# Samaretas/global-motion-estimation

Measured on AMD Instinct MI355X. Metric: frame-pairs/s + achieved HBM GB/s, 720x480 bs=16 sw=16 exhaustive, higher is better.
Workload: dtype u8; 1 GPU; 720x480 synthetic luma, bs=16 sw=16 exhaustive MAE (BASELINE configs[1]); frame_distance=1, streams_per_gpu=1, collective=none, exchange=none in this run, multi_gpu_measured_by_builder=False

## Files before the change

global-motion-estimation_amd/csrc/bbme_sea.hip:

```cpp
#include "bbme_sea_common.h"

namespace {

using namespace sea;

constexpr int GUARD_NONE = 0, GUARD_ROWS = 1, GUARD_ALL = 2;
constexpr uint32_t PENALTY = 1u << 17;
constexpr uint32_t FIRST_INVALID_KEY = 65536u << 13;
constexpr uint32_t FIRST_INVALID_BOUND = FIRST_INVALID_KEY >> 13;
__device__ __forceinline__ uint32_t pair_u16(uint32_t t, uint32_t b, bool odd)
{
    return __builtin_amdgcn_perm(b, t, odd ? 0x07060302u : 0x05040100u);
}
template <bool VERT>
__device__ __forceinline__ void candidate_pairs(uint32_t tl, uint32_t tr, uint32_t bl, uint32_t br, bool odd, uint32_t* first, uint32_t* second)
{
    *first = VERT ? pair_u16(tl, bl, odd) : pair_u16(tl, tr, odd);
    *second = VERT ? pair_u16(tr, br, odd) : pair_u16(bl, br, odd);
}
template <int R, int GUARD, bool VERT>
__device__ __forceinline__ void lower_bounds(const uint64_t* sp0, int XQ, int prow, int q, uint32_t pa, uint32_t pb,
                                             int lo_r, int hi_r, int lo_c, int hi_c, uint32_t (&pmin)[R])
{
    constexpr bool SKIP = GUARD == GUARD_ALL && R >= 4;
#pragma unroll
    for (int k = 0; k < R; ++k) pmin[k] = 0xFFFFFFFFu;
    constexpr uint32_t penalty = PENALTY;
    uint32_t seed[R];
#pragma unroll
    for (int i = 0; i < R; ++i) {
        const int ri = prow * R + i;
        seed[i] = (GUARD == GUARD_NONE || SKIP || (ri >= lo_r && ri <= hi_r)) ? 0u : penalty;
    }
    const int nlo = lo_c - q * 4 * R, nhi = hi_c - q * 4 * R;
    const uint64_t* top = sp0;
    const uint64_t* bot = sp0 + 8 * XQ;
#pragma unroll
    for (int i = 0; i < R; ++i) {
        const int ri = prow * R + i;
        if (!SKIP || (ri >= lo_r && ri <= hi_r)) {
            uint64_t t[R + 2], b[R + 2];
#pragma unroll
            for (int k = 0; k < R + 2; ++k) { t[k] = top[k]; b[k] = bot[k]; }
            if constexpr (SKIP || !VERT) {
#pragma unroll
                for (int k = 0; k < R; ++k) {
                    if (SKIP && (4 * k > nhi || 4 * k + 3 < nlo)) continue;
#pragma unroll
                    for (int e = 0; e < 4; ++e) {
                        if (SKIP && (4 * k + e < nlo || 4 * k + e > nhi)) continue;
                        const int sh = 32 * (e >> 1);
                        uint32_t first, second;
                        candidate_pairs<VERT>((uint32_t)(t[k] >> sh), (uint32_t)(t[k + 2] >> sh), (uint32_t)(b[k] >> sh), (uint32_t)(b[k + 2] >> sh), e & 1, &first, &second);
                        const uint32_t start = (GUARD != GUARD_ALL || SKIP || 4 * k + e <= nhi) ? seed[i] : penalty;
                        pmin[k] = min(pmin[k], __builtin_amdgcn_sad_u16(first, pa, __builtin_amdgcn_sad_u16(second, pb, start)));
                    }
                }
            } else {
                uint32_t vp[R + 2][4];
#pragma unroll
                for (int k = 0; k < R; ++k) {
#pragma unroll
                    for (int m = (k < 2 ? k : k + 2); m <= k + 2; m += 2)
#pragma unroll
                        for (int e = 0; e < 4; ++e)
                            vp[m][e] = pair_u16((uint32_t)(t[m] >> (32 * (e >> 1))), (uint32_t)(b[m] >> (32 * (e >> 1))), e & 1);
                    uint32_t lb[4];
#pragma unroll
                    for (int e = 0; e < 4; ++e) {
                        const uint32_t start = (GUARD != GUARD_ALL || 4 * k + e <= nhi) ? seed[i] : penalty;
                        lb[e] = __builtin_amdgcn_sad_u16(vp[k][e], pa, __builtin_amdgcn_sad_u16(vp[k + 2][e], pb, start));
                    }
                    pmin[k] = min(min(pmin[k], lb[0]), lb[1]);
                    pmin[k] = min(min(pmin[k], lb[2]), lb[3]);
                }
            }
        }
        top += XQ;
        bot += XQ;
    }
    if constexpr (GUARD != GUARD_NONE && !SKIP) {
#pragma unroll
        for (int k = 0; k < R; ++k)
            if (pmin[k] >= FIRST_INVALID_BOUND || (GUARD == GUARD_ALL && 4 * k < nlo)) pmin[k] = 0xFFFFFFFFu;
    }
}

template <int R, bool VERT>
__device__ __forceinline__ int min_bound_candidate(const uint64_t* s8blk, int XQ, int NC, int bl, uint32_t mb, uint32_t pa, uint32_t pb,
                                                   int lo_r, int hi_r, int lo_c, int hi_c, int lane)
{
    const int col0 = (bl & 3) * 4 * R, row0 = (bl >> 2) * R;
    const uint16_t* tab = (const uint16_t*)(s8blk + row0 * XQ + (bl & 3) * R);
    int loc = 0;
    bool found = false;
#pragma unroll
    for (int base = 0; base < 4 * R * R; base += 64) {
        const int l = base + lane;
        const int ce = l / R, li = l - ce * R;
        bool hit = false;
        if (4 * R * R - base >= 64 || l < 4 * R * R) {
            const uint16_t* p = tab + li * 4 * XQ + ce;
            uint32_t first, second;
            candidate_pairs<VERT>(p[0], p[8], p[32 * XQ], p[32 * XQ + 8], false, &first, &second);
            const uint32_t lb = __builtin_amdgcn_sad_u16(first, pa, __builtin_amdgcn_sad_u16(second, pb, 0u));
            const int ci = col0 + ce, ri = row0 + li;
            hit = lb == mb && ci >= lo_c && ci <= hi_c && ri >= lo_r && ri <= hi_r;
        }
        const unsigned long long m = __ballot(hit);
        if (!found && m) {
            loc = base + __builtin_ctzll(m);
            found = true;
        }
    }
    const int ce = loc / R, li = loc - ce * R;
    return (col0 + ce) * NC + row0 + li;
}

template <int R>
__device__ __forceinline__ uint32_t eval_patch_quad(const SeaGeo& d, int H, int W, const uint32_t* win, const uint32_t* anchor, uint32_t ent,
                                                    bool active, int sub, int trow, int bcol0, int NC)
{
    const int w2 = ent >> 25, l2 = (ent >> 19) & 63, k2 = (ent >> 16) & 7;
    const int wr2 = div_small(w2, d.magic_tc), wc2 = w2 - wr2 * d.tc;
    const int prow2 = l2 >> 2, q2 = l2 & 3;
    uint64_t acc[R];
#pragma unroll
    for (int i = 0; i < R; ++i) acc[i] = 0;
    if (active) {
        const uint32_t* lrow = win + (16 * wr2 + prow2 * R + 4 * sub) * d.pitch_dw + wc2 * 4 + q2 * R + k2;
        const uint32_t* an = anchor + w2 * ANCHOR_STRIDE + 16 * sub;
#pragma unroll
        for (int t = 0; t < R + 3; ++t) {
            uint64_t w[4];
#pragma unroll
            for (int s = 0; s < 4; ++s) w[s] = *(const u64_a4*)(lrow + t * d.pitch_dw + s);
#pragma unroll
            for (int i = 0; i < R; ++i) {
                const int a = t - i;
                if (a < 0 || a > 3) continue;
                const u32x4 ar = *(const u32x4*)(an + a * 4);
#pragma unroll
                for (int j = 0; j < 4; ++j)
                    acc[i] = __builtin_amdgcn_qsad_pk_u16_u8(w[j], ar[j], acc[i]);
            }
        }
    }
#pragma unroll
    for (int i = 0; i < R; ++i) {
        uint32_t lo = (uint32_t)acc[i], hi = (uint32_t)(acc[i] >> 32);
        lo += (uint32_t)__builtin_amdgcn_update_dpp(0, (int)lo, 0xB1, 0xF, 0xF, false);
        hi += (uint32_t)__builtin_amdgcn_update_dpp(0, (int)hi, 0xB1, 0xF, 0xF, false);
        lo += (uint32_t)__builtin_amdgcn_update_dpp(0, (int)lo, 0x4E, 0xF, 0xF, false);
        hi += (uint32_t)__builtin_amdgcn_update_dpp(0, (int)hi, 0x4E, 0xF, 0xF, false);
        asm volatile("" : "+v"(lo), "+v"(hi));
        acc[i] = ((uint64_t)hi << 32) | lo;
    }
    uint32_t key = 0xFFFFFFFFu;
    if (active) {
        const int c02 = (bcol0 + wc2) * 16, r02 = (trow * d.tr + wr2) * 16;
        const int lo_c = max(0, d.sw - c02), hi_c = min(NC - 1, W - 16 - c02 + d.sw);
        const int lo_r2 = max(0, d.sw - r02), hi_r2 = min(NC - 1, H - 16 - r02 + d.sw);
        const bool rows_inside2 = NC == 16 * R && lo_r2 == 0 && hi_r2 == NC - 1;
        const int ci = q2 * 4 * R + 4 * k2 + sub, ri0 = prow2 * R;
        const uint32_t shift = (uint32_t)(sub & 1) * 16u;
        if (rows_inside2 && lo_c == 0 && hi_c == NC - 1) {
#pragma unroll
            for (int i = 0; i < R; ++i) {
                const uint32_t word = (sub & 2) ? (uint32_t)(acc[i] >> 32) : (uint32_t)acc[i];
                const uint32_t sad = __builtin_amdgcn_ubfe(word, shift, 16u);
                key = min(key, (sad << 13) + (uint32_t)i);
            }
            key += (uint32_t)(ci * NC + ri0);
        } else if (ci >= lo_c && ci <= hi_c) {
#pragma unroll
            for (int i = 0; i < R; ++i) {
                const int ri = ri0 + i;
                if (ri < lo_r2 || ri > hi_r2) continue;
                const uint32_t word = (sub & 2) ? (uint32_t)(acc[i] >> 32) : (uint32_t)acc[i];
                const uint32_t sad = __builtin_amdgcn_ubfe(word, shift, 16u);
                key = min(key, (sad << 13) | (uint32_t)(ci * NC + ri));
            }
        }
        key = min(key, (uint32_t)__builtin_amdgcn_update_dpp(-1, (int)key, 0xB1, 0xF, 0xF, false));
        key = min(key, (uint32_t)__builtin_amdgcn_update_dpp(-1, (int)key, 0x4E, 0xF, 0xF, false));
    }
    return key;
}

template <int R, bool FIXED, bool VERT>
__device__ __forceinline__ bool tile_phases(const SeaGeo& d, uint32_t* lds, const Layout& L, int pair, int trow, int bcol0,
                                            uint32_t mine, uint32_t pa, uint32_t pb, int tid, int tile_id)
{
    constexpr bool E4 = R >= 3;
    const int T = blockDim.x;
    const int NC = 2 * d.sw + 16, XQ = d.xq;
    uint32_t* win = lds + L.win;
    uint32_t* anchor = lds + L.anchor;
    uint32_t* best = lds + L.best;
    uint32_t* count = lds + L.count;
    uint64_t* s8 = (uint64_t*)(lds + L.s8);
    uint32_t* work = lds + L.work;
    const int wave = __builtin_amdgcn_readfirstlane(tid >> 6);
    const int lane = tid & 63;
    const SeaArgs c = launch_args();
    const WaveBlock wb = wave_block(d, c, trow, bcol0, wave);
    const int brow = wb.brow, bcol = wb.bcol;
    const bool wave_ok = wb.ok;
    const int r0 = brow * 16, c0 = bcol * 16;
    const int prow = lane >> 2, q = lane & 3;

    box_sums8<R, FIXED>(d, win, s8, tid);
    __syncthreads();

    const int lo_r = max(0, d.sw - r0), hi_r = min(NC - 1, c->H - 16 - r0 + d.sw);
    const bool rows_inside = NC == 16 * R && lo_r == 0 && hi_r == NC - 1;
    uint32_t ub_key = 0xFFFFFFFFu;
    if (wave_ok) {
        const int lo_c = max(0, d.sw - c0), hi_c = min(NC - 1, c->W - 16 - c0 + d.sw);
        uint32_t pmin[R];
        const uint64_t* s8blk = s8 + 16 * wb.wr * XQ + wb.wc * 4;
        const uint64_t* sp0 = s8blk + prow * R * XQ + q * R;
        const bool cols_inside = NC == 16 * R && lo_c == 0 && hi_c == NC - 1;
        if (rows_inside && cols_inside)
            lower_bounds<R, GUARD_NONE, VERT>(sp0, XQ, prow, q, pa, pb, lo_r, hi_r, lo_c, hi_c, pmin);
        else if (R <= 3 && cols_inside)
            lower_bounds<R, GUARD_ROWS, VERT>(sp0, XQ, prow, q, pa, pb, lo_r, hi_r, lo_c, hi_c, pmin);
        else
            lower_bounds<R, GUARD_ALL, VERT>(sp0, XQ, prow, q, pa, pb, lo_r, hi_r, lo_c, hi_c, pmin);
        const uint32_t first_idx = (uint32_t)((q * 4 * R) * NC + prow * R);
        uint32_t pkd[R], lane_min = 0xFFFFFFFFu;
#pragma unroll
        for (int k = 0; k < R; ++k) {
            pkd[k] = (pmin[k] << 13) | (first_idx + (uint32_t)(4 * k * NC));
            lane_min = min(lane_min, pmin[k]);
        }
        const uint32_t lane_lb = lane_min << 13;
        uint32_t lb_key = lane_min != 0xFFFFFFFFu ? lane_lb + ((uint32_t)lane << 7) : 0xFFFFFFFFu;
        lb_key = wave_min_u32(lb_key);
        {
            const int idx1 = min_bound_candidate<R, VERT>(s8blk, XQ, NC, (int)(lb_key >> 7) & 63, lb_key >> 13, pa, pb,
                                                          lo_r, hi_r, lo_c, hi_c, lane);
            const int idx0 = d.sw * NC + d.sw;
            const int arow = lane >> 2, aj = lane & 3;
            uint32_t packed = 0;
#pragma unroll
            for (int which = 0; which < 2; ++which) {
                const int idx = which ? idx1 : idx0;
                const int ci = idx / NC, ri = idx - ci * NC;
                const int byte = wb.wc * 16 + ci + 4 * aj;
                const uint32_t* p = win + (16 * wb.wr + ri + arow) * d.pitch_dw + (byte >> 2);
                const uint32_t v = __builtin_amdgcn_alignbyte(p[1], p[0], (uint32_t)byte & 3u);
                packed += __builtin_amdgcn_sad_u8(v, mine, 0u) << (16 * which);
            }
            packed = wave_sum_u32(packed);
            ub_key = min(((packed & 0xFFFFu) << 13) | (uint32_t)idx0, ((packed >> 16) << 13) | (uint32_t)idx1);
            const int idxp = (int)(best[2 * wave + 1] & 0x1FFFu);
            const int cip = idxp / NC, rip = idxp - cip * NC;
            if (idxp != idx0 && idxp != idx1 && cip >= lo_c && cip <= hi_c && rip >= lo_r && rip <= hi_r) {
                const int byte = wb.wc * 16 + cip + 4 * aj;
                const uint32_t* p = win + (16 * wb.wr + rip + arow) * d.pitch_dw + (byte >> 2);
                const uint32_t v = __builtin_amdgcn_alignbyte(p[1], p[0], (uint32_t)byte & 3u);
                const uint32_t sadp = wave_sum_u32(__builtin_amdgcn_sad_u8(v, mine, 0u));
                ub_key = min(ub_key, (sadp << 13) | (uint32_t)idxp);
            }
        }
        uint32_t own_lim = 0;
        int n_w = 0;
        if constexpr (E4) {
            const int engage = c->engage;
            if (c->quota > 0 && __popcll(__ballot(lane_lb < ub_key)) > engage / 3) {
#pragma unroll
                for (int k = 0; k < R; ++k) n_w += __popcll(__ballot(pkd[k] < ub_key));
                if (n_w > engage) {
                    own_lim = first_round_limit(c, lb_key >> 13, ub_key >> 13, 13, [&](uint32_t lim) {
                        int c = 0;
#pragma unroll
                        for (int k = 0; k < R; ++k) c += __popcll(__ballot(pkd[k] < lim));
                        return c;
                    });
                    own_lim = min(own_lim, ub_key);
                    uint32_t* own = lds + L.own + 16 * wave;
                    int base_rank = 0;
                    uint32_t listed_here = 0;
#pragma unroll
                    for (int k = 0; k < R; ++k) {
                        const bool sel = pkd[k] < own_lim;
                        const unsigned long long m = __ballot(sel);
                        const int rank = base_rank + (int)__builtin_amdgcn_mbcnt_hi((uint32_t)(m >> 32), __builtin_amdgcn_mbcnt_lo((uint32_t)m, 0u));
                        if (sel && rank < 16) {
                            own[rank] = ((uint32_t)wave << 25) | ((uint32_t)lane << 19) | ((uint32_t)k << 16) | (pkd[k] >> 13);
                            listed_here |= 1u << k;
                        }
                        base_rank += __popcll(m);
                    }
                    const int n_own = min(base_rank, 16);
                    const bool act = (lane >> 2) < n_own;
                    const uint32_t ent = act ? own[lane >> 2] : 0u;
                    uint32_t key = eval_patch_quad<R>(d, c->H, c->W, win, anchor, ent, act, lane & 3, trow, bcol0, NC);
                    ub_key = min(ub_key, wave_min_u32(key));
#pragma unroll
                    for (int k = 0; k < R; ++k)
                        if (listed_here & (1u << k)) pkd[k] = 0xFFFFFFFFu;
                    if (lane == 0) atomicAdd(count + 5, (uint32_t)n_own);
                }
            }
        }
        if (lane == 0) best[2 * wave] = ub_key;
#pragma unroll
        for (int k = 0; k < R; ++k)
            if (pkd[k] < ub_key) {
                const uint32_t slot = atomicAdd(count, 1u);
                work[slot] = ((uint32_t)wave << 25) | ((uint32_t)lane << 19) | ((uint32_t)k << 16) | (pkd[k] >> 13);
            }
        if (own_lim) {
            int pushed = 0;
#pragma unroll
            for (int k = 0; k < R; ++k) pushed += __popcll(__ballot(pkd[k] < ub_key));
            if (lane == 0) atomicAdd(count + 4, (uint32_t)(n_w - pushed));
        }
    }
    __syncthreads();
    const SeaArgs ce = launch_args();
    if (ce->redo_list && (int)*count > ce->redo_threshold) {
        if (tid == 0) push_redo(ce, tile_id, (int)(blockIdx.x & 7));
        return true;
    }
    const int H = ce->H, W = ce->W;

    if constexpr (E4) {
        const int n = (int)*count;
        const int sub = lane & 3;
        for (int base = 0; base < n; base += T / 4) {
            const int e = base + (tid >> 2);
            bool active = e < n;
            uint32_t ent = 0;
            if (active) ent = work[e];
            const int w2 = ent >> 25, l2 = (ent >> 19) & 63, k2 = (ent >> 16) & 7;
            const int wr2 = div_small(w2, d.magic_tc), wc2 = w2 - wr2 * d.tc;
            const int prow2 = l2 >> 2, q2 = l2 & 3;
            active = active && (((ent & 0xFFFFu) << 13) | (uint32_t)((q2 * 4 * R + 4 * k2) * NC + prow2 * R)) < best[2 * w2];
            uint64_t acc[R];
    #pragma unroll
            for (int i = 0; i < R; ++i) acc[i] = 0;
            if (active) {
                const uint32_t* lrow = win + (16 * wr2 + prow2 * R + 4 * sub) * d.pitch_dw + wc2 * 4 + q2 * R + k2;
                const uint32_t* an = anchor + w2 * ANCHOR_STRIDE + 16 * sub;
    #pragma unroll
                for (int t = 0; t < R + 3; ++t) {
                    uint64_t w[4];
    #pragma unroll
                    for (int s = 0; s < 4; ++s) w[s] = *(const u64_a4*)(lrow + t * d.pitch_dw + s);
    #pragma unroll
                    for (int i = 0; i < R; ++i) {
                        const int a = t - i;
                        if (a < 0 || a > 3) continue;
                        const u32x4 ar = *(const u32x4*)(an + a * 4);
    #pragma unroll
                        for (int j = 0; j < 4; ++j)
                            acc[i] = __builtin_amdgcn_qsad_pk_u16_u8(w[j], ar[j], acc[i]);
                    }
                }
            }
    #pragma unroll
            for (int i = 0; i < R; ++i) {
                uint32_t lo = (uint32_t)acc[i], hi = (uint32_t)(acc[i] >> 32);
                lo += (uint32_t)__builtin_amdgcn_update_dpp(0, (int)lo, 0xB1, 0xF, 0xF, false);
                hi += (uint32_t)__builtin_amdgcn_update_dpp(0, (int)hi, 0xB1, 0xF, 0xF, false);
                lo += (uint32_t)__builtin_amdgcn_update_dpp(0, (int)lo, 0x4E, 0xF, 0xF, false);
                hi += (uint32_t)__builtin_amdgcn_update_dpp(0, (int)hi, 0x4E, 0xF, 0xF, false);
                asm volatile("" : "+v"(lo), "+v"(hi));
                acc[i] = ((uint64_t)hi << 32) | lo;
            }
            if (active) {
                const int c02 = (bcol0 + wc2) * 16, r02 = (trow * d.tr + wr2) * 16;
                const int lo_c = max(0, d.sw - c02), hi_c = min(NC - 1, W - 16 - c02 + d.sw);
                const int lo_r2 = max(0, d.sw - r02), hi_r2 = min(NC - 1, H - 16 - r02 + d.sw);
                const bool rows_inside2 = NC == 16 * R && lo_r2 == 0 && hi_r2 == NC - 1;
                const int ci = q2 * 4 * R + 4 * k2 + sub, ri0 = prow2 * R;
                const uint32_t shift = (uint32_t)(sub & 1) * 16u;
                uint32_t key = 0xFFFFFFFFu;
                if (rows_inside2 && lo_c == 0 && hi_c == NC - 1) {
    #pragma unroll
                    for (int i = 0; i < R; ++i) {
                        const uint32_t word = (sub & 2) ? (uint32_t)(acc[i] >> 32) : (uint32_t)acc[i];
                        const uint32_t sad = __builtin_amdgcn_ubfe(word, shift, 16u);
                        key = min(key, (sad << 13) + (uint32_t)i);
                    }
                    key += (uint32_t)(ci * NC + ri0);
                } else if (ci >= lo_c && ci <= hi_c) {
    #pragma unroll
                    for (int i = 0; i < R; ++i) {
                        const int ri = ri0 + i;
                        if (ri < lo_r2 || ri > hi_r2) continue;
                        const uint32_t word = (sub & 2) ? (uint32_t)(acc[i] >> 32) : (uint32_t)acc[i];
                        const uint32_t sad = __builtin_amdgcn_ubfe(word, shift, 16u);
                        key = min(key, (sad << 13) | (uint32_t)(ci * NC + ri));
                    }
                }
                key = min(key, (uint32_t)__builtin_amdgcn_update_dpp(-1, (int)key, 0xB1, 0xF, 0xF, false));
                key = min(key, (uint32_t)__builtin_amdgcn_update_dpp(-1, (int)key, 0x4E, 0xF, 0xF, false));
                if (sub == 0 && key != 0xFFFFFFFFu) atomicMin(&best[2 * w2], key);
            }
            __syncthreads();
        }
    } else {
        const int n = (int)*count;
        for (int base = 0; base < n; base += T) {
            const int e = base + tid;
            bool active = e < n;
            uint32_t ent = 0;
            if (active) {
                ent = work[e];
                const uint32_t first = (uint32_t)(((int)((ent >> 19) & 3) * 4 * R + 4 * (int)((ent >> 16) & 7)) * NC + (int)((ent >> 21) & 15) * R);
                active = (((ent & 0xFFFFu) << 13) | first) < best[2 * (ent >> 25)];
            }
            if (active) {
                const int w2 = ent >> 25, l2 = (ent >> 19) & 63, k2 = (ent >> 16) & 7;
                const int wr2 = div_small(w2, d.magic_tc), wc2 = w2 - wr2 * d.tc;
                const int prow2 = l2 >> 2, q2 = l2 & 3;
                const uint32_t* lrow = win + (16 * wr2 + prow2 * R) * d.pitch_dw + wc2 * 4 + q2 * R + k2;
                const uint32_t* an = anchor + w2 * ANCHOR_STRIDE;
                uint64_t acc[R];
    #pragma unroll
                for (int i = 0; i < R; ++i) acc[i] = 0;
    #pragma unroll
                for (int t = 0; t < R + 15; ++t) {
                    uint64_t w[4];
    #pragma unroll
                    for (int s = 0; s < 4; ++s) w[s] = *(const u64_a4*)(lrow + t * d.pitch_dw + s);
    #pragma unroll
                    for (int i = 0; i < R; ++i) {
                        const int a = t - i;
                        if (a < 0 || a > 15) continue;
                        const u32x4 ar = *(const u32x4*)(an + a * 4);
    #pragma unroll
                        for (int j = 0; j < 4; ++j)
                            acc[i] = __builtin_amdgcn_qsad_pk_u16_u8(w[j], ar[j], acc[i]);
                    }
                }
                const int c02 = (bcol0 + wc2) * 16, r02 = (trow * d.tr + wr2) * 16;
                const int lo_c = max(0, d.sw - c02), hi_c = min(NC - 1, W - 16 - c02 + d.sw);
                const int lo_r2 = max(0, d.sw - r02), hi_r2 = min(NC - 1, H - 16 - r02 + d.sw);
                const bool rows_inside2 = NC == 16 * R && lo_r2 == 0 && hi_r2 == NC - 1;
                const int ci0 = q2 * 4 * R + 4 * k2, ri0 = prow2 * R;
                uint32_t key = 0xFFFFFFFFu;
                if (rows_inside2 && lo_c == 0 && hi_c == NC - 1) {
    #pragma unroll
                    for (int e4 = 0; e4 < 4; ++e4)
    #pragma unroll
                        for (int i = 0; i < R; ++i) {
                            const uint32_t sad = (uint32_t)(acc[i] >> (16 * e4)) & 0xFFFFu;
                            key = min(key, (sad << 13) + (uint32_t)(e4 * NC + i));
                        }
                    key += (uint32_t)(ci0 * NC + ri0);
                } else {
    #pragma unroll
                    for (int e4 = 0; e4 < 4; ++e4) {
                        const int ci = ci0 + e4;
                        if (ci < lo_c || ci > hi_c) continue;
    #pragma unroll
                        for (int i = 0; i < R; ++i) {
                            const int ri = ri0 + i;
                            if (ri < lo_r2 || ri > hi_r2) continue;
                            const uint32_t sad = (uint32_t)(acc[i] >> (16 * e4)) & 0xFFFFu;
                            key = min(key, (sad << 13) | (uint32_t)(ci * NC + ri));
                        }
                    }
                }
                if (key != 0xFFFFFFFFu) atomicMin(&best[2 * w2], key);
            }
            __syncthreads();
        }

    }
    if (wave_ok && lane == 0) {
        const int idx = (int)(best[2 * wave] & 0x1FFF);
        const int ci = idx / NC, ri = idx - ci * NC;
        int32_t* o = ce->mf + (((long long)pair * ce->nbr + brow) * ce->nbc + bcol) * 2;
        o[0] = ci - d.sw;
        o[1] = ri - d.sw;
        best[2 * wave + 1] = (uint32_t)idx;
    }
    return false;
}

template <int R, bool FIXED = false, bool VERT = true>
struct MaeTile {
    struct Pre { uint32_t pa, pb; };
    static __device__ __forceinline__ Pre prep(uint32_t* lds, const Layout& L, int wave, int lane, bool wave_ok, uint32_t mine)
    {
        Pre p = { 0, 0 };
        if (wave_ok) {
            lds[L.anchor + wave * ANCHOR_STRIDE + lane] = mine;
            uint32_t a01, a23;
            anchor_quadrants(mine, &a01, &a23);
            p.pa = VERT ? pair_u16(a01, a23, false) : a01;
            p.pb = VERT ? pair_u16(a01, a23, true) : a23;
        }
        return p;
    }
    static __device__ __forceinline__ bool phases(const SeaGeo& d, uint32_t* lds, const Layout& L, int pair, int trow, int bcol0,
                                                  uint32_t mine, const Pre& p, int tid, int tile_id)
    {
        return tile_phases<R, FIXED, VERT>(d, lds, L, pair, trow, bcol0, mine, p.pa, p.pb, tid, tile_id);
    }
    static __device__ __forceinline__ int probe_word(const Layout& L, int wave) { return L.best + 2 * wave + 1; }
};

template <int R>
__global__ void __launch_bounds__(1024) k_exh_sea16(SeaDev d)
{
    extern __shared__ uint32_t lds[];
    const SeaGeo g = d;
    one_tile<MaeTile<R>>(g, lds, layout_of(g, R));
}

constexpr bool vertical_pairs(int R, int NV) { return !(R == 5 && NV == 16); }

template <int R, int NV, int GEO = 0>
__global__ void __launch_bounds__(1024, (R <= 3 ? 8 : 6)) k_exh_sea16p(SeaDev d)
{
    extern __shared__ uint32_t lds[];
    SeaGeo g = d;
    fix_geometry<R, GEO>(g);
    const Layout L = layout_of(g, R);
    if ((threadIdx.x & 63) == 0) lds[L.best + 2 * (threadIdx.x >> 6) + 1] = (uint32_t)(g.sw * (2 * g.sw + 16) + g.sw);
    persistent_tiles<NV, MaeTile<R, GEO != 0, vertical_pairs(R, NV)>>(g, lds, L);
}

struct MaeLaunch {
    static constexpr const char* persistent_name = "k_exh_sea16p";
    static constexpr const char* one_tile_name = "k_exh_sea16";
    static int no_plan()
    {
        gme_set_error("search window too large for LDS");
        return GME_ERR_ARG;
    }
    static void tables(SeaDev& d, const BbmeJob&) { d.sqbox = nullptr; d.sqbox_stride = 0; }
// ... 37 lines not shown
```

global-motion-estimation_amd/csrc/bbme_sea_common.h:

```cpp
#pragma once
#include <stdlib.h>

#include "gme_internal.h"

namespace sea {

constexpr double SHARE_WEIGHT = 0.5;

struct SeaGeo {
    int sw;
    int tr, tc, nb;
    uint32_t magic_tc;
    int pitch_dw, win_rows;
    int s8_rows;
    int rstep;
    uint32_t magic_pitch;
    uint32_t magic_xq;
    int xq;
};

struct SeaDev : SeaGeo {
    unsigned long long magic_wpp;
    unsigned long long magic_wpr;
    const uint8_t* cur;
// ... 68 lines not shown
{
    Layout l{};
    l.win = 0;
    l.anchor = (win_rows * pitch_dw + 3) & ~3;
    l.best = (l.anchor + nb * ANCHOR_STRIDE + 1) & ~1;
    l.count = l.best + 2 * nb;
    l.a2 = l.count + 8;
    l.prev = l.a2 + nb;
    l.own = l.prev + nb;
    l.s8 = (l.own + 16 * nb + 1) & ~1;
    l.work = l.s8 + 2 * s8_rows * xq;
    l.total = l.work + nb * 64 * R;
    return l;
}

__device__ __forceinline__ Layout layout_of(const SeaGeo& d, int R)
{
    return make_layout(R, d.nb, d.win_rows, d.pitch_dw, d.xq, d.s8_rows);
}

struct WaveBlock {
    int wr, wc;
    int brow, bcol;
    bool ok;
};
__device__ __forceinline__ WaveBlock wave_block(const SeaGeo& d, SeaArgs c, int trow, int bcol0, int wave)
{
    WaveBlock b;
    b.wr = div_small(wave, d.magic_tc);
    b.wc = wave - b.wr * d.tc;
    b.brow = trow * d.tr + b.wr;
    b.bcol = bcol0 + b.wc;
    b.ok = b.bcol < c->nbc && b.brow < c->nbr;
    return b;
}

__device__ __forceinline__ void stage_window(const SeaGeo& d, SeaArgs c, uint32_t* win, const uint8_t* cur, int bcol0, int r0)
{
    const int pitch = c->pitch, H = c->H;
    const int gx0 = bcol0 * 16 - d.sw, gy0 = r0 - d.sw;
    const int rstep = d.rstep;
    const int row0 = div_small((int)threadIdx.x, d.magic_pitch), dw = (int)threadIdx.x - row0 * d.pitch_dw;
    const int gx = gx0 + 4 * dw;
    const bool colok = gx >= 0 && gx < pitch;
    if (row0 < rstep) {
        const uint8_t* src = cur + (long long)(gy0 + row0) * pitch + gx;
        const long long sstep = (long long)rstep * pitch;
        uint32_t* dst = win + threadIdx.x;
        const int dstep = rstep * d.pitch_dw;
        for (int row = row0; row < d.win_rows; row += 4 * rstep, src += 4 * sstep, dst += 4 * dstep) {
            uint32_t v[4];
#pragma unroll
            for (int u = 0; u < 4; ++u) {
                const int gy = gy0 + row + u * rstep;
                v[u] = 0;
                if (colok && row + u * rstep < d.win_rows && gy >= 0 && gy < H) v[u] = *(const uint32_t*)(src + u * sstep);
            }
#pragma unroll
            for (int u = 0; u < 4; ++u)
                if (row + u * rstep < d.win_rows) dst[u * dstep] = v[u];
        }
    }
}

template <int CH, bool FIXED>
__device__ __forceinline__ void box_sums8_ch(const SeaGeo& d, const uint32_t* win, uint64_t* s8, int tid, int need)
{
    static_assert((CH + 7) * 1020 < 65536, "cumulative 4-byte sums must fit 16 bits");
    const int XQ = d.xq;
    const int wave = __builtin_amdgcn_readfirstlane(tid >> 6), lane = tid & 63;
    const int SL = XQ == need ? XQ + 1 : XQ;
    const bool wide = SL > 64;
    const uint32_t magic_sl = XQ == need ? div_magic(SL) : d.magic_xq;
    const int SEG = wide ? 1 : div_small(64, magic_sl);
    const int units = wide ? 8 * div_small(XQ + 62, div_magic(63)) : 8;
    const int ls = wide ? 0 : div_small(lane, magic_sl);
    const int RB = FIXED ? 254 / d.pitch_dw + 1 : 1;
    for (int u = wave * SEG; u < units; u += d.nb * SEG) {
        const int ch = wide ? (u & 7) : u + ls;
        const int sq = wide ? (u >> 3) * 63 + lane : lane - ls * SL;
        const bool active = wide ? sq < SL : (ls < SEG && ch < 8);
        const bool stores = active && sq < XQ && (!wide || lane < 63);
        int pi = active ? (ch * CH) * d.pitch_dw + sq : 0, oi = (ch * CH) * XQ + sq;
        uint64_t ring[8], acc = 0;
#pragma unroll
        for (int r = 0; r < CH + 7; ++r) {
            if constexpr (FIXED) {
                if (r > 0 && r % RB == 0) {
                    pi += RB * d.pitch_dw;
                    asm volatile("" : "+v"(pi));
                }
                acc = __builtin_amdgcn_qsad_pk_u16_u8(*(const u64_a4*)(win + pi + (r % RB) * d.pitch_dw), 0u, acc);
            } else {
                acc = __builtin_amdgcn_qsad_pk_u16_u8(*(const u64_a4*)(win + pi), 0u, acc);
                pi += d.pitch_dw;
                asm volatile("" : "+v"(pi));
            }
            if (r >= 7) {
                uint32_t lo = (uint32_t)acc, hi = (uint32_t)(acc >> 32);
                if (r >= 8) { lo -= (uint32_t)ring[r & 7]; hi -= (uint32_t)(ring[r & 7] >> 32); }
                lo += SEA_DPP(lo, 0x130);
                hi += SEA_DPP(hi, 0x130);
                asm volatile("" : "+v"(lo), "+v"(hi));
                if constexpr (FIXED) {
                    if (stores) s8[oi + (r - 7) * XQ] = ((uint64_t)hi << 32) | lo;
                } else {
                    if (stores) s8[oi] = ((uint64_t)hi << 32) | lo;
                    oi += XQ;
                    asm volatile("" : "+v"(oi));
                }
            }
            ring[r & 7] = acc;
        }
    }
}

template <int R, bool FIXED>
__device__ __forceinline__ void box_sums8(const SeaGeo& d, const uint32_t* win, uint64_t* s8, int tid)
{
    const int need = 4 * R + 4 * (d.tc - 1) + 2;
    if (d.tr == 1) box_sums8_ch<2 * R + 1, FIXED>(d, win, s8, tid, need);
    else if (d.tr == 2) box_sums8_ch<2 * R + 3, FIXED>(d, win, s8, tid, need);
    else box_sums8_ch<2 * R + 7, FIXED>(d, win, s8, tid, need);
}

__device__ __forceinline__ void anchor_quadrants(uint32_t mine, uint32_t* a01, uint32_t* a23)
{
    uint32_t s = __builtin_amdgcn_sad_u8(mine, 0u, 0u);
    s += SEA_DPP(s, 0xB1);
    s += SEA_DPP(s, 0x124);
    s += SEA_DPP(s, 0x128);
    const uint32_t q0 = (uint32_t)__builtin_amdgcn_readlane((int)s, 0) + (uint32_t)__builtin_amdgcn_readlane((int)s, 16);
    const uint32_t q1 = (uint32_t)__builtin_amdgcn_readlane((int)s, 2) + (uint32_t)__builtin_amdgcn_readlane((int)s, 18);
    const uint32_t q2 = (uint32_t)__builtin_amdgcn_readlane((int)s, 32) + (uint32_t)__builtin_amdgcn_readlane((int)s, 48);
    const uint32_t q3 = (uint32_t)__builtin_amdgcn_readlane((int)s, 34) + (uint32_t)__builtin_amdgcn_readlane((int)s, 50);
    *a01 = q0 | (q1 << 16);
    *a23 = q2 | (q3 << 16);
}

constexpr int box_conflicts(int xq, int R)
{
    int worst = 0, hits[64] = {};
    for (int b = 0; b < 64; ++b) hits[b] = 0;
    for (int prow = 0; prow < 8; ++prow)
        for (int q = 0; q < 4; ++q) {
            const int dw = 2 * ((prow * R) * xq + q * R);
            ++hits[dw & 63]; ++hits[(dw + 1) & 63];
        }
    for (int b = 0; b < 64; ++b) worst = hits[b] > worst ? hits[b] : worst;
    return worst;
}
constexpr int pick_xq(int need, int R)
{
    int best = need, best_c = 1 << 30;
    for (int x = need; x < need + 12; ++x) {
        const int c = box_conflicts(x, R);
        if (c < best_c) { best_c = c; best = x; }
    }
    return best;
}

constexpr int pick_pitch(int need, int R)
{
    int best_p = need, best_c = 1 << 30;
    for (int p = need; p < need + 16; ++p) {
        int quad = 0, seen[32] = {};
        for (int i = 0; i < 32; ++i) seen[i] = 0;
        for (int sub = 0; sub < 4; ++sub) { quad += seen[(4 * sub * p) & 31]; ++seen[(4 * sub * p) & 31]; quad += seen[(4 * sub * p + 1) & 31]; }
        int probe = 0;
        for (int i = 0; i < 32; ++i) seen[i] = 0;
        for (int row = 0; row < 8; ++row)
            for (int dw = 0; dw < 4; ++dw) probe += seen[(row * p + dw) & 31]++;
        const int c = 64 * quad + probe + 2 * (p - need);
        if (c < best_c) { best_c = c; best_p = p; }
    }
    (void)R;
    return best_p;
}

struct Shape { int tr, tc, pitch, xq; size_t bytes; };
// ... 43 lines not shown
        for (int tr = 1; tr <= 4; tr *= 2)
            for (int tc = 1; tc * tr <= 16; ++tc) {
                if (tc > nbc || (tr > 1 && tr > nbr) || (pass == 0 && (tr * tc) % 4 != 0)) continue;
                const Shape s = shape(tr, tc);
                if (s.bytes > 160 * 1024 || s.pitch >= 256 || s.xq >= 256) continue;
                const int nb = tr * tc;
                int wgs = (int)((160 * 1024) / (s.bytes + 1024));
                if (wgs * nb > wave_cap) wgs = wave_cap / nb;
                if (wgs < 1) wgs = 1;
                const int waves = wgs * nb;
                const double cover = ((double)nbc / (((nbc + tc - 1) / tc) * tc)) * ((double)nbr / (((nbr + tr - 1) / tr) * tr));
                const double simd_eff = (double)nb / (4 * ((nb + 3) / 4));
                const double area = (double)(16 * tr + 2 * sw + 15) * (16 * tc + 2 * sw + 15) / nb;
                const double own = (double)(2 * sw + 31) * (2 * sw + 31);
                const double share = 1.0 + SHARE_WEIGHT * (1.0 - area / own);
                const double together = wgs == 1 ? 0.93 : 1.0 + 0.03 * ((wgs > 4 ? 4 : wgs) - 2);
                const double tall = tr == 4 ? 0.95 : 1.0;
                const double score = waves * cover * simd_eff * share * together * tall + nb * 1e-3;
                if (score > best_score) { best_score = score; best = s; }
            }
    if (best_score < 0) return false;
    d->tr = best.tr; d->tc = best.tc; d->nb = best.tr * best.tc;
    d->magic_tc = div_magic(d->tc);
    d->wg_per_row = (nbc + d->tc - 1) / d->tc;
    d->tile_rows = (nbr + d->tr - 1) / d->tr;
    d->wg_per_pair = d->wg_per_row * d->tile_rows;
    d->win_rows = 16 * R + 15 + 16 * (d->tr - 1);
    d->s8_rows = 16 * R + 8 + 16 * (d->tr - 1);
    d->pitch_dw = best.pitch; d->xq = best.xq;
    *lds_bytes = best.bytes;
    d->rstep = 64 * d->nb / d->pitch_dw;
    d->magic_pitch = div_magic(d->pitch_dw);
    d->magic_xq = div_magic(d->xq);
    d->magic_wpp = div_magic40(d->wg_per_pair);
    d->magic_wpr = div_magic40(d->wg_per_row);
    return d->rstep >= 1;
}

constexpr int SEA_DEFAULT_QUOTA = 16, SEA_DEFAULT_BISECT = 5, SEA_DEFAULT_ENGAGE = 24;
constexpr int REDO_BURST = 15;
constexpr double REDO_DEFAULT_FRAC = 0.75;

__device__ __forceinline__ void push_redo(SeaArgs c, int tile_in_xcd, int xcd)
{
    uint32_t* status = c->status;
    const uint32_t slot = atomicAdd(status + GME_STATUS_REDO, 1u);
    c->redo_list[slot] = ((uint32_t)tile_in_xcd << 3) | (uint32_t)xcd;
    atomicAdd(status + GME_STATUS_STATS + 16 * xcd + 1, 1u);
}

template <class Below>
__device__ __forceinline__ uint32_t first_round_limit(SeaArgs c, uint32_t lo, uint32_t hi, int shift, Below below)
{
    const int bisect = c->bisect, quota = c->quota;
    if (bisect < 0) return (lo + ((hi - lo) >> -bisect) + 1) << shift;
    for (int s = 0; s < bisect && lo < hi; ++s) {
        const uint32_t mid = (lo + hi) >> 1;
        if ((int)below((mid + 1) << shift) > quota) hi = mid; else lo = mid;
    }
    return (lo + 1) << shift;
}

__device__ __forceinline__ int tile_number(const SeaGeo& d, SeaArgs c, int pair, int trow, int bcol0)
{
    return (pair >> 3) * c->wg_per_pair + trow * c->wg_per_row + div_small(bcol0, d.magic_tc);
}


template <class Kern>
__device__ __forceinline__ void one_tile(const SeaGeo& d, uint32_t* lds, const Layout L)
{
    const SeaArgs c = launch_args();
    int pair, trow, bcol0;
    if (!locate(d, c, &pair, &trow, &bcol0)) return;
    const int wave = __builtin_amdgcn_readfirstlane(threadIdx.x >> 6);
    const int lane = threadIdx.x & 63;
    const long long plane = (long long)pair * c->plane_stride;
    stage_window(d, c, lds + L.win, c->cur + plane, bcol0, trow * d.tr * 16);
    uint32_t mine = 0;
    const WaveBlock wb = wave_block(d, c, trow, bcol0, wave);
    if (wb.ok) {
        const int pitch = c->pitch;
        const uint8_t* aptr = c->prev + plane + (long long)(wb.brow * 16) * pitch + wb.bcol * 16;
        mine = *(const uint32_t*)(aptr + (long long)(lane >> 2) * pitch + (lane & 3) * 4);
    }
    const typename Kern::Pre pre = Kern::prep(lds, L, wave, lane, wb.ok, mine);
    if (lane == 0) lds[Kern::probe_word(L, wave)] = (uint32_t)(d.sw * (2 * d.sw + 16) + d.sw);
    if (threadIdx.x == 0) { lds[L.count] = 0; lds[L.count + 4] = 0; lds[L.count + 5] = 0; lds[L.count + 7] = 0; }
    __syncthreads();
    Kern::phases(d, lds, L, pair, trow, bcol0, mine, pre, (int)threadIdx.x, tile_number(d, c, pair, trow, bcol0));
    if (threadIdx.x == 0) {
        uint32_t* stats = launch_args()->status + GME_STATUS_STATS + 16 * (blockIdx.x & 7);
        atomicAdd(stats, lds[L.count] + lds[L.count + 5]);
        atomicAdd(stats + 2, lds[L.count] + lds[L.count + 4]);
    }
}

__device__ __forceinline__ int tiles_of_xcd(SeaArgs c, int xcd) { return ((c->pairs - xcd + 7) >> 3) * c->wg_per_pair; }
__device__ __forceinline__ uint32_t* tile_counter(SeaArgs c, int xcd) { return c->dynamic ? c->status + GME_STATUS_TILECTR + 16 * xcd : nullptr; }

template <int NV, class Kern>
__device__ __forceinline__ void persistent_tiles(const SeaGeo& d, uint32_t* lds, const Layout L)
{
    const int xcd = blockIdx.x & 7;
    int tile = blockIdx.x >> 3;
    if (tile >= tiles_of_xcd(launch_args(), xcd)) return;
    int tid_carried = (int)threadIdx.x;
    auto opaque_tid = [&]() {
        asm volatile("" : "+v"(tid_carried));
        return tid_carried;
    };

    uint32_t wv[NV], an_next = 0;
    int pair = 0, trow = 0, bcol0 = 0;
    auto fetch = [&](int t, int tid) {
        const SeaArgs c = launch_args();
        const int wave = __builtin_amdgcn_readfirstlane(tid >> 6), lane = tid & 63;
        const int row0 = div_small(tid, d.magic_pitch), dw = tid - row0 * d.pitch_dw;
        const int lp = (int)(((unsigned long long)(unsigned)t * c->magic_wpp) >> 40);
        const int wg = t - lp * c->wg_per_pair;
        const int wpr = c->wg_per_row;
        trow = (int)(((unsigned long long)(unsigned)wg * c->magic_wpr) >> 40);
        bcol0 = (wg - trow * wpr) * d.tc;
        pair = lp * 8 + xcd;
        const int pitch = c->pitch;
        const long long plane = (long long)pair * c->plane_stride;
        const uint8_t* cur = c->cur + plane;
        const unsigned long long cur_bits = (unsigned long long)cur;
        const __amdgpu_buffer_rsrc_t rs = __builtin_amdgcn_make_buffer_rsrc(
            (void*)(((unsigned long long)(unsigned)__builtin_amdgcn_readfirstlane((int)(cur_bits >> 32)) << 32) |
                    (unsigned)__builtin_amdgcn_readfirstlane((int)cur_bits)),
            (short)0, __builtin_amdgcn_readfirstlane(c->H * pitch), 0x00020000);
        const int gx0 = bcol0 * 16 - d.sw + 4 * dw, gy0 = trow * d.tr * 16 - d.sw + row0;
        const bool colok = row0 < d.rstep && gx0 >= 0 && gx0 < pitch;
        int outside = (int)0x80000000;
        asm volatile("" : "+v"(outside));
        const int off0 = colok ? gy0 * pitch + gx0 : outside;
        const int sstep = d.rstep * pitch;
#pragma unroll
        for (int u = 0; u < NV; ++u)
            wv[u] = (uint32_t)__builtin_amdgcn_raw_buffer_load_b32(rs, colok ? off0 + u * sstep : off0, 0, 0);
        an_next = 0;
        const WaveBlock wb = wave_block(d, c, trow, bcol0, wave);
        if (wb.ok) {
            const uint8_t* aptr = c->prev + plane + (long long)(wb.brow * 16) * pitch + wb.bcol * 16;
            an_next = *(const uint32_t*)(aptr + (long long)(lane >> 2) * pitch + (lane & 3) * 4);
        }
    };
    fetch(tile, opaque_tid());
    uint32_t drawn = 0;
    if (opaque_tid() == 0) {
        if (uint32_t* ctr = tile_counter(launch_args(), xcd)) drawn = atomicInc(ctr, 0xFFFFFFFFu);
        lds[L.count] = 0; lds[L.count + 3] = 0; lds[L.count + 4] = 0; lds[L.count + 5] = 0; lds[L.count + 7] = 0;
    }
    uint32_t stat_scored = 0, stat_listed = 0;
    for (;;) {
        const int tid = opaque_tid();
        const int wave = __builtin_amdgcn_readfirstlane(tid >> 6), lane = tid & 63;
        const int gx = launch_groups_x(launch_args()) >> 3;
        {
            const int row0 = div_small(tid, d.magic_pitch);
            if (row0 < d.rstep) {
                uint32_t* dst = lds + L.win + tid;
                const int dstep = d.rstep * d.pitch_dw;
#pragma unroll
                for (int u = 0; u < NV; ++u)
                    if (row0 + u * d.rstep < d.win_rows) dst[u * dstep] = wv[u];
            }
        }
        const int pair_c = pair, trow_c = trow, bcol0_c = bcol0, tile_c = tile;
        const uint32_t mine = an_next;
        const typename Kern::Pre pre = Kern::prep(lds, L, wave, lane, wave_block(d, launch_args(), trow_c, bcol0_c, wave).ok, mine);
        if (tid == 0) {
            const uint32_t listed = lds[L.count], c2_off = lds[L.count + 4], c2_scored = lds[L.count + 5];
            stat_scored += listed + c2_scored;
            stat_listed += listed + c2_off;
            lds[L.count] = 0; lds[L.count + 4] = 0; lds[L.count + 5] = 0; lds[L.count + 7] = 0;
            lds[L.count + 1] = (uint32_t)gx + drawn;
        }
        __syncthreads();
        bool more, dynamic;
        {
            const SeaArgs c = launch_args();
            dynamic = c->dynamic != 0;
            tile = dynamic ? (int)lds[L.count + 1] : tile + (launch_groups_x(c) >> 3);
            more = tile < tiles_of_xcd(c, xcd);
            if (more) {
                fetch(tile, tid);
                if (dynamic && tid == 0) drawn = atomicInc(c->status + GME_STATUS_TILECTR + 16 * xcd, 0xFFFFFFFFu);
            }
        }
        if (!Kern::phases(d, lds, L, pair_c, trow_c, bcol0_c, mine, pre, tid, tile_c)) {
            if (tid == 0) lds[L.count + 3] = 0;
        } else if (dynamic && wave == 0) {
            const int streak = (int)lds[L.count + 3];
            const int burst = streak == 0 ? 0 : streak == 1 ? 3 : streak == 2 ? 7 : REDO_BURST;
            if (burst) {
                const SeaArgs c = launch_args();
                uint32_t got = 0;
                if (lane >= 1 && lane <= burst) got = atomicAdd(c->status + GME_STATUS_TILECTR + 16 * xcd, 1u);
                const int t = (launch_groups_x(c) >> 3) + (int)(lane == 0 ? drawn : got);
                if (lane < burst && t < tiles_of_xcd(c, xcd)) push_redo(c, t, xcd);
                drawn = (uint32_t)__builtin_amdgcn_readlane((int)got, __builtin_amdgcn_readfirstlane(burst));
            }
            if (lane == 0) lds[L.count + 3] = (uint32_t)(streak + 1);
        }
        if (!more) break;
    }
    if (opaque_tid() == 0) {
        uint32_t* stats = launch_args()->status + GME_STATUS_STATS + 16 * xcd;
        atomicAdd(stats, stat_scored + lds[L.count] + lds[L.count + 5]);
        atomicAdd(stats + 2, stat_listed + lds[L.count] + lds[L.count + 4]);
    }
}

struct PersistPlan { bool use; bool dynamic; long long g; int nv; };
inline PersistPlan plan_persistent(const SeaDev& d, size_t lds_bytes, int pairs, int cu_count)
{
    PersistPlan p;
    const long long tiles_x = (((long long)pairs + 7) / 8) * d.wg_per_pair;
    p.nv = (d.win_rows + d.rstep - 1) / d.rstep;
    const char* pmode = getenv("GME_SEA_PERSIST");
    const int pm = pmode ? atoi(pmode) : -1;
    int per_cu = (int)((160 * 1024) / (lds_bytes + 1024));
    if (per_cu * d.nb > 32) per_cu = 32 / d.nb;
    if (per_cu < 1) per_cu = 1;
    p.g = (long long)per_cu * cu_count / 8;
    const bool can = tiles_x < (1ll << 21) && d.wg_per_pair < (1 << 18) && p.nv <= 16 && p.g >= 1;
    p.use = can && (pm > 0 || (pm < 0 && tiles_x >= 4 * p.g));
// ... 77 lines not shown
```

Baseline: 614,400 frame-pairs/s.

## Aggregate work-list pushes per wave and precompute interior flags in entries

Replaces per-lane LDS atomicAdd pushes into the work list with one wave-level ds_add_rtn and mbcnt-based slot assignment. It also encodes an interior flag in each work entry so the evaluation stages skip recomputing border bounds, and cheapens the wave-row division when the tile width is a power of two. Separately, it prefetches rows in the integral/sum precompute ring loop, leaves accumulators undefined for inactive lanes, and simplifies buffer-load offsets. The cost is more register pressure from the prefetch array and a slight reliance on out-of-range buffer loads returning zero.

```diff
diff --git a/global-motion-estimation_amd/csrc/bbme_sea.hip b/global-motion-estimation_amd/csrc/bbme_sea.hip
--- a/global-motion-estimation_amd/csrc/bbme_sea.hip
+++ b/global-motion-estimation_amd/csrc/bbme_sea.hip
@@ -8,6 +8,25 @@
 constexpr uint32_t PENALTY = 1u << 17;
 constexpr uint32_t FIRST_INVALID_KEY = 65536u << 13;
 constexpr uint32_t FIRST_INVALID_BOUND = FIRST_INVALID_KEY >> 13;
+__device__ __forceinline__ uint32_t lds_add_rtn(uint32_t* p, uint32_t v)
+{
+    uint32_t old;
+    const uint32_t addr = (uint32_t)(uintptr_t)(__attribute__((address_space(3))) uint32_t*)p;
+    asm volatile("ds_add_rtn_u32 %0, %1, %2\n\ts_waitcnt lgkmcnt(0)" : "=v"(old) : "v"(addr), "v"(v) : "memory");
+    return old;
+}
+constexpr uint32_t ENT_INTERIOR = 1u << 29;
+__device__ __forceinline__ int wave_row(const SeaGeo& d, int w)
+{
+    if (__builtin_constant_p(d.tc) && (d.tc & (d.tc - 1)) == 0) return w >> __builtin_ctz((unsigned)d.tc);
+    return div_small(w, d.magic_tc);
+}
+__device__ __forceinline__ uint64_t any_u64()
+{
+    uint32_t lo, hi;
+    asm volatile("" : "=v"(lo), "=v"(hi));
+    return ((uint64_t)hi << 32) | lo;
+}
 __device__ __forceinline__ uint32_t pair_u16(uint32_t t, uint32_t b, bool odd)
 {
     return __builtin_amdgcn_perm(b, t, odd ? 0x07060302u : 0x05040100u);
@@ -121,13 +140,15 @@
 __device__ __forceinline__ uint32_t eval_patch_quad(const SeaGeo& d, int H, int W, const uint32_t* win, const uint32_t* anchor, uint32_t ent,
                                                     bool active, int sub, int trow, int bcol0, int NC)
 {
-    const int w2 = ent >> 25, l2 = (ent >> 19) & 63, k2 = (ent >> 16) & 7;
-    const int wr2 = div_small(w2, d.magic_tc), wc2 = w2 - wr2 * d.tc;
+    const int w2 = (ent >> 25) & 15, l2 = (ent >> 19) & 63, k2 = (ent >> 16) & 7;
+    const int wr2 = wave_row(d, w2), wc2 = w2 - wr2 * d.tc;
     const int prow2 = l2 >> 2, q2 = l2 & 3;
     uint64_t acc[R];
 #pragma unroll
-    for (int i = 0; i < R; ++i) acc[i] = 0;
+    for (int i = 0; i < R; ++i) acc[i] = any_u64();
     if (active) {
+#pragma unroll
+        for (int i = 0; i < R; ++i) acc[i] = 0;
         const uint32_t* lrow = win + (16 * wr2 + prow2 * R + 4 * sub) * d.pitch_dw + wc2 * 4 + q2 * R + k2;
         const uint32_t* an = anchor + w2 * ANCHOR_STRIDE + 16 * sub;
 #pragma unroll
@@ -158,13 +179,9 @@
     }
     uint32_t key = 0xFFFFFFFFu;
     if (active) {
-        const int c02 = (bcol0 + wc2) * 16, r02 = (trow * d.tr + wr2) * 16;
-        const int lo_c = max(0, d.sw - c02), hi_c = min(NC - 1, W - 16 - c02 + d.sw);
-        const int lo_r2 = max(0, d.sw - r02), hi_r2 = min(NC - 1, H - 16 - r02 + d.sw);
-        const bool rows_inside2 = NC == 16 * R && lo_r2 == 0 && hi_r2 == NC - 1;
         const int ci = q2 * 4 * R + 4 * k2 + sub, ri0 = prow2 * R;
         const uint32_t shift = (uint32_t)(sub & 1) * 16u;
-        if (rows_inside2 && lo_c == 0 && hi_c == NC - 1) {
+        if (ent & ENT_INTERIOR) {
 #pragma unroll
             for (int i = 0; i < R; ++i) {
                 const uint32_t word = (sub & 2) ? (uint32_t)(acc[i] >> 32) : (uint32_t)acc[i];
@@ -172,11 +189,14 @@
                 key = min(key, (sad << 13) + (uint32_t)i);
             }
             key += (uint32_t)(ci * NC + ri0);
-        } else if (ci >= lo_c && ci <= hi_c) {
+        } else {
+            const int c02 = (bcol0 + wc2) * 16, r02 = (trow * d.tr + wr2) * 16;
+            const int lo_c = max(0, d.sw - c02), hi_c = min(NC - 1, W - 16 - c02 + d.sw);
+            const int lo_r2 = max(0, d.sw - r02), hi_r2 = min(NC - 1, H - 16 - r02 + d.sw);
 #pragma unroll
             for (int i = 0; i < R; ++i) {
                 const int ri = ri0 + i;
-                if (ri < lo_r2 || ri > hi_r2) continue;
+                if (ci < lo_c || ci > hi_c || ri < lo_r2 || ri > hi_r2) continue;
                 const uint32_t word = (sub & 2) ? (uint32_t)(acc[i] >> 32) : (uint32_t)acc[i];
                 const uint32_t sad = __builtin_amdgcn_ubfe(word, shift, 16u);
                 key = min(key, (sad << 13) | (uint32_t)(ci * NC + ri));
@@ -229,6 +249,7 @@
         else
             lower_bounds<R, GUARD_ALL, VERT>(sp0, XQ, prow, q, pa, pb, lo_r, hi_r, lo_c, hi_c, pmin);
         const uint32_t first_idx = (uint32_t)((q * 4 * R) * NC + prow * R);
+        const uint32_t ent0 = (rows_inside && cols_inside ? ENT_INTERIOR : 0u) | ((uint32_t)wave << 25) | ((uint32_t)lane << 19);
         uint32_t pkd[R], lane_min = 0xFFFFFFFFu;
 #pragma unroll
         for (int k = 0; k < R; ++k) {
@@ -289,7 +310,7 @@
                         const unsigned long long m = __ballot(sel);
                         const int rank = base_rank + (int)__builtin_amdgcn_mbcnt_hi((uint32_t)(m >> 32), __builtin_amdgcn_mbcnt_lo((uint32_t)m, 0u));
                         if (sel && rank < 16) {
-                            own[rank] = ((uint32_t)wave << 25) | ((uint32_t)lane << 19) | ((uint32_t)k << 16) | (pkd[k] >> 13);
+                            own[rank] = ent0 | ((uint32_t)k << 16) | (pkd[k] >> 13);
                             listed_here |= 1u << k;
                         }
                         base_rank += __popcll(m);
@@ -307,18 +328,26 @@
             }
         }
         if (lane == 0) best[2 * wave] = ub_key;
-#pragma unroll
-        for (int k = 0; k < R; ++k)
-            if (pkd[k] < ub_key) {
-                const uint32_t slot = atomicAdd(count, 1u);
-                work[slot] = ((uint32_t)wave << 25) | ((uint32_t)lane << 19) | ((uint32_t)k << 16) | (pkd[k] >> 13);
-            }
-        if (own_lim) {
-            int pushed = 0;
-#pragma unroll
-            for (int k = 0; k < R; ++k) pushed += __popcll(__ballot(pkd[k] < ub_key));
-            if (lane == 0) atomicAdd(count + 4, (uint32_t)(n_w - pushed));
-        }
+        unsigned long long pushes[R];
+        int pushed = 0;
+#pragma unroll
+        for (int k = 0; k < R; ++k) {
+            pushes[k] = __ballot(pkd[k] < ub_key);
+            pushed += __popcll(pushes[k]);
+        }
+        if (pushed) {
+            uint32_t base = 0;
+            if (lane == 0) base = lds_add_rtn(count, (uint32_t)pushed);
+            uint32_t slot = (uint32_t)__builtin_amdgcn_readfirstlane((int)base);
+#pragma unroll
+            for (int k = 0; k < R; ++k) {
+                if (pkd[k] < ub_key)
+                    work[__builtin_amdgcn_mbcnt_hi((uint32_t)(pushes[k] >> 32), __builtin_amdgcn_mbcnt_lo((uint32_t)pushes[k], slot))] =
+                        ent0 | ((uint32_t)k << 16) | (pkd[k] >> 13);
+                slot += (uint32_t)__popcll(pushes[k]);
+            }
+        }
+        if (own_lim && lane == 0) atomicAdd(count + 4, (uint32_t)(n_w - pushed));
     }
     __syncthreads();
     const SeaArgs ce = launch_args();
@@ -336,14 +365,17 @@
             bool active = e < n;
             uint32_t ent = 0;
             if (active) ent = work[e];
-            const int w2 = ent >> 25, l2 = (ent >> 19) & 63, k2 = (ent >> 16) & 7;
-            const int wr2 = div_small(w2, d.magic_tc), wc2 = w2 - wr2 * d.tc;
+            const int w2 = (ent >> 25) & 15, l2 = (ent >> 19) & 63, k2 = (ent >> 16) & 7;
+            const int wr2 = wave_row(d, w2), wc2 = w2 - wr2 * d.tc;
             const int prow2 = l2 >> 2, q2 = l2 & 3;
-            active = active && (((ent & 0xFFFFu) << 13) | (uint32_t)((q2 * 4 * R + 4 * k2) * NC + prow2 * R)) < best[2 * w2];
+            const uint32_t first2 = (uint32_t)((q2 * 4 * R + 4 * k2) * NC + prow2 * R);
+            active = active && (((ent & 0xFFFFu) << 13) | first2) < best[2 * w2];
             uint64_t acc[R];
     #pragma unroll
-            for (int i = 0; i < R; ++i) acc[i] = 0;
+            for (int i = 0; i < R; ++i) acc[i] = any_u64();
             if (active) {
+    #pragma unroll
+                for (int i = 0; i < R; ++i) acc[i] = 0;
                 const uint32_t* lrow = win + (16 * wr2 + prow2 * R + 4 * sub) * d.pitch_dw + wc2 * 4 + q2 * R + k2;
                 const uint32_t* an = anchor + w2 * ANCHOR_STRIDE + 16 * sub;
     #pragma unroll
@@ -373,26 +405,25 @@
                 acc[i] = ((uint64_t)hi << 32) | lo;
             }
             if (active) {
-                const int c02 = (bcol0 + wc2) * 16, r02 = (trow * d.tr + wr2) * 16;
-                const int lo_c = max(0, d.sw - c02), hi_c = min(NC - 1, W - 16 - c02 + d.sw);
-                const int lo_r2 = max(0, d.sw - r02), hi_r2 = min(NC - 1, H - 16 - r02 + d.sw);
-                const bool rows_inside2 = NC == 16 * R && lo_r2 == 0 && hi_r2 == NC - 1;
                 const int ci = q2 * 4 * R + 4 * k2 + sub, ri0 = prow2 * R;
                 const uint32_t shift = (uint32_t)(sub & 1) * 16u;
                 uint32_t key = 0xFFFFFFFFu;
-                if (rows_inside2 && lo_c == 0 && hi_c == NC - 1) {
+                if (ent & ENT_INTERIOR) {
     #pragma unroll
                     for (int i = 0; i < R; ++i) {
                         const uint32_t word = (sub & 2) ? (uint32_t)(acc[i] >> 32) : (uint32_t)acc[i];
                         const uint32_t sad = __builtin_amdgcn_ubfe(word, shift, 16u);
                         key = min(key, (sad << 13) + (uint32_t)i);
                     }
-                    key += (uint32_t)(ci * NC + ri0);
-                } else if (ci >= lo_c && ci <= hi_c) {
+                    key += first2 + (uint32_t)(sub * NC);
+                } else {
+                    const int c02 = (bcol0 + wc2) * 16, r02 = (trow * d.tr + wr2) * 16;
+                    const int lo_c = max(0, d.sw - c02), hi_c = min(NC - 1, W - 16 - c02 + d.sw);
+                    const int lo_r2 = max(0, d.sw - r02), hi_r2 = min(NC - 1, H - 16 - r02 + d.sw);
     #pragma unroll
                     for (int i = 0; i < R; ++i) {
                         const int ri = ri0 + i;
-                        if (ri < lo_r2 || ri > hi_r2) continue;
+                        if (ci < lo_c || ci > hi_c || ri < lo_r2 || ri > hi_r2) continue;
                         const uint32_t word = (sub & 2) ? (uint32_t)(acc[i] >> 32) : (uint32_t)acc[i];
                         const uint32_t sad = __builtin_amdgcn_ubfe(word, shift, 16u);
                         key = min(key, (sad << 13) | (uint32_t)(ci * NC + ri));
@@ -413,11 +444,11 @@
             if (active) {
                 ent = work[e];
                 const uint32_t first = (uint32_t)(((int)((ent >> 19) & 3) * 4 * R + 4 * (int)((ent >> 16) & 7)) * NC + (int)((ent >> 21) & 15) * R);
-                active = (((ent & 0xFFFFu) << 13) | first) < best[2 * (ent >> 25)];
+                active = (((ent & 0xFFFFu) << 13) | first) < best[2 * ((ent >> 25) & 15)];
             }
             if (active) {
-                const int w2 = ent >> 25, l2 = (ent >> 19) & 63, k2 = (ent >> 16) & 7;
-                const int wr2 = div_small(w2, d.magic_tc), wc2 = w2 - wr2 * d.tc;
+                const int w2 = (ent >> 25) & 15, l2 = (ent >> 19) & 63, k2 = (ent >> 16) & 7;
+                const int wr2 = wave_row(d, w2), wc2 = w2 - wr2 * d.tc;
                 const int prow2 = l2 >> 2, q2 = l2 & 3;
                 const uint32_t* lrow = win + (16 * wr2 + prow2 * R) * d.pitch_dw + wc2 * 4 + q2 * R + k2;
                 const uint32_t* an = anchor + w2 * ANCHOR_STRIDE;
@@ -439,13 +470,9 @@
                             acc[i] = __builtin_amdgcn_qsad_pk_u16_u8(w[j], ar[j], acc[i]);
                     }
                 }
-                const int c02 = (bcol0 + wc2) * 16, r02 = (trow * d.tr + wr2) * 16;
-                const int lo_c = max(0, d.sw - c02), hi_c = min(NC - 1, W - 16 - c02 + d.sw);
-                const int lo_r2 = max(0, d.sw - r02), hi_r2 = min(NC - 1, H - 16 - r02 + d.sw);
-                const bool rows_inside2 = NC == 16 * R && lo_r2 == 0 && hi_r2 == NC - 1;
                 const int ci0 = q2 * 4 * R + 4 * k2, ri0 = prow2 * R;
                 uint32_t key = 0xFFFFFFFFu;
-                if (rows_inside2 && lo_c == 0 && hi_c == NC - 1) {
+                if (ent & ENT_INTERIOR) {
     #pragma unroll
                     for (int e4 = 0; e4 < 4; ++e4)
     #pragma unroll
@@ -455,6 +482,9 @@
                         }
                     key += (uint32_t)(ci0 * NC + ri0);
                 } else {
+                    const int c02 = (bcol0 + wc2) * 16, r02 = (trow * d.tr + wr2) * 16;
+                    const int lo_c = max(0, d.sw - c02), hi_c = min(NC - 1, W - 16 - c02 + d.sw);
+                    const int lo_r2 = max(0, d.sw - r02), hi_r2 = min(NC - 1, H - 16 - r02 + d.sw);
     #pragma unroll
                     for (int e4 = 0; e4 < 4; ++e4) {
                         const int ci = ci0 + e4;
diff --git a/global-motion-estimation_amd/csrc/bbme_sea_common.h b/global-motion-estimation_amd/csrc/bbme_sea_common.h
--- a/global-motion-estimation_amd/csrc/bbme_sea_common.h
+++ b/global-motion-estimation_amd/csrc/bbme_sea_common.h
@@ -174,20 +174,28 @@
         const bool active = wide ? sq < SL : (ls < SEG && ch < 8);
         const bool stores = active && sq < XQ && (!wide || lane < 63);
         int pi = active ? (ch * CH) * d.pitch_dw + sq : 0, oi = (ch * CH) * XQ + sq;
-        uint64_t ring[8], acc = 0;
+        constexpr int ROWS = CH + 7, STEP = FIXED ? 8 : 1, AHEAD = FIXED ? 16 : 1;
+        uint64_t ring[8], acc = 0, w[ROWS];
+        int read = 0;
 #pragma unroll
-        for (int r = 0; r < CH + 7; ++r) {
-            if constexpr (FIXED) {
-                if (r > 0 && r % RB == 0) {
-                    pi += RB * d.pitch_dw;
-                    asm volatile("" : "+v"(pi));
+        for (int r = 0; r < ROWS; ++r) {
+            if (r % STEP == 0) {
+#pragma unroll
+                for (; read < ROWS && read < r + AHEAD; ++read) {
+                    if constexpr (FIXED) {
+                        if (read > 0 && read % RB == 0) {
+                            pi += RB * d.pitch_dw;
+                            asm volatile("" : "+v"(pi));
+                        }
+                        w[read] = *(const u64_a4*)(win + pi + (read % RB) * d.pitch_dw);
+                    } else {
+                        w[read] = *(const u64_a4*)(win + pi);
+                        pi += d.pitch_dw;
+                        asm volatile("" : "+v"(pi));
+                    }
                 }
-                acc = __builtin_amdgcn_qsad_pk_u16_u8(*(const u64_a4*)(win + pi + (r % RB) * d.pitch_dw), 0u, acc);
-            } else {
-                acc = __builtin_amdgcn_qsad_pk_u16_u8(*(const u64_a4*)(win + pi), 0u, acc);
-                pi += d.pitch_dw;
-                asm volatile("" : "+v"(pi));
             }
+            acc = __builtin_amdgcn_qsad_pk_u16_u8(w[r], 0u, acc);
             if (r >= 7) {
                 uint32_t lo = (uint32_t)acc, hi = (uint32_t)(acc >> 32);
                 if (r >= 8) { lo -= (uint32_t)ring[r & 7]; hi -= (uint32_t)(ring[r & 7] >> 32); }
@@ -397,7 +405,7 @@
     if (wb.ok) {
         const int pitch = c->pitch;
         const uint8_t* aptr = c->prev + plane + (long long)(wb.brow * 16) * pitch + wb.bcol * 16;
-        mine = *(const uint32_t*)(aptr + (long long)(lane >> 2) * pitch + (lane & 3) * 4);
+        mine = *(const uint32_t*)(aptr + (uint32_t)((lane >> 2) * pitch + (lane & 3) * 4));
     }
     const typename Kern::Pre pre = Kern::prep(lds, L, wave, lane, wb.ok, mine);
     if (lane == 0) lds[Kern::probe_word(L, wave)] = (uint32_t)(d.sw * (2 * d.sw + 16) + d.sw);
@@ -454,12 +462,12 @@
         const int sstep = d.rstep * pitch;
 #pragma unroll
         for (int u = 0; u < NV; ++u)
-            wv[u] = (uint32_t)__builtin_amdgcn_raw_buffer_load_b32(rs, colok ? off0 + u * sstep : off0, 0, 0);
+            wv[u] = (uint32_t)__builtin_amdgcn_raw_buffer_load_b32(rs, off0 + u * sstep, 0, 0);
         an_next = 0;
         const WaveBlock wb = wave_block(d, c, trow, bcol0, wave);
         if (wb.ok) {
             const uint8_t* aptr = c->prev + plane + (long long)(wb.brow * 16) * pitch + wb.bcol * 16;
-            an_next = *(const uint32_t*)(aptr + (long long)(lane >> 2) * pitch + (lane & 3) * 4);
+            an_next = *(const uint32_t*)(aptr + (uint32_t)((lane >> 2) * pitch + (lane & 3) * 4));
         }
     };
     fetch(tile, opaque_tid());
```

After: 629,800 frame-pairs/s, median of 6. 2.5% higher.
